# goktug97/estorch

Measured on NVIDIA H100. Metric: generations/sec at pop=4096, 1M-param MLP, higher is better.
Workload: dtype f32 (fp32-equivalent: evaluate GEMMs on wgmma with fp16 operands = 11-bit significand, TF32 class, each weight formed in fp32 from fp32 theta + the exactly-16-bit noise value and rounded once, f32 accumulate, f32 bias/loss; f32 ranks, reduction, Adam)

## Files before the change

estorch_b200/csrc/estk_eval_mlp_tc.cu:

```cuda
#include "estk_tc.cuh"
#include <type_traits>

namespace {

constexpr int kRows = 64;
constexpr int kTileN = 128;
constexpr int kHBlockBytes = kRows * kBlockK * 2;
constexpr int kHBytes = (kMaxW / kBlockK) * kHBlockBytes;
constexpr int kStageBytes = kTileN * kBlockK * 2;
constexpr int kStages = 5;
constexpr int kCluster = 4;
constexpr int kProdWarps = 8, kProdGroups = 4, kProdGroupWarps = kProdWarps / kProdGroups;
constexpr int kPT = 32 * kProdGroupWarps;
constexpr int kThreadsTC = 128 + 32 * kProdWarps;
static_assert(kProdGroups <= kStages, "parity waits need kProdGroups <= kStages");
constexpr int kItemsPT = kTileN / kCluster * (kBlockK / 8) / kPT;
constexpr int kTgtBatch = 4;
constexpr int kModeBF16 = 0, kModeBF16S = 1, kModeF16 = 2;

struct EvalTCParams {
  estk_mlp_desc desc;
  const float* theta;
  const float* table;
  const uint16_t* theta16;
  const uint16_t* table16;
  const int64_t* offsets;
  const int32_t* order;
  int pairs;
  float sigma;
  const float* obs;
  const float* target;
  int B, chunks;
  float* ret_plus;
  float* ret_minus;
  float* bc_plus;
  float* bc_minus;
  int bc_obs, bc_dim;
  float* partial;
  unsigned int* counters;
  float* centre_out;
  int n_centre;
  int n_tasks;
  int n_signs;
  int mode;
#ifdef ESTK_TC_PROFILE
  unsigned long long* prof;
#endif
};

#ifdef ESTK_TC_PROFILE
enum { kPrFull, kPrMma, kPrDrain, kPrLayer, kPrTask, kPrLoad, kPrEmpty, kPrForm, kPrBuckets };
unsigned long long* g_prof_buf = nullptr;
#define ESTK_PROF_DECL long long pr_[kPrBuckets] = {}; long long pr_t_ = clock64();
#define ESTK_PROF(b) do { const long long n_ = clock64(); pr_[b] += n_ - pr_t_; pr_t_ = n_; } while (0)
#else
#define ESTK_PROF_DECL
#define ESTK_PROF(b) do {} while (0)
#endif

struct Layer { int K, N; int64_t wbase, bbase; };

struct TaskId { int slot, sgn, chunk; bool centre; };
__device__ __forceinline__ TaskId decode_task(const EvalTCParams& p, int task, bool all_centre) {
  TaskId t;
  if (task < p.n_centre) { t.slot = 0; t.sgn = 0; t.chunk = task; t.centre = true; return t; }
  const int q = task - p.n_centre;
  t.chunk = q % p.chunks;
  t.sgn = (q / p.chunks) % p.n_signs;
  t.slot = q / (p.chunks * p.n_signs);
  t.centre = all_centre;
  return t;
}

template <int MODE>
__global__ void __launch_bounds__(kThreadsTC, 1) eval_mlp_tc_kernel(const EvalTCParams p) {
  constexpr bool S16 = (MODE == kModeBF16S), F16 = (MODE == kModeF16);
  extern __shared__ __align__(1024) uint8_t smem_raw[];
  uint8_t* smem = reinterpret_cast<uint8_t*>((reinterpret_cast<uintptr_t>(smem_raw) + 1023) & ~uintptr_t(1023));
  uint8_t* sH = smem;
  uint8_t* sB = sH + 2 * kHBytes;
  float* sBias = reinterpret_cast<float*>(sB + kStages * kStageBytes);
  uint64_t* bar_full = reinterpret_cast<uint64_t*>(sBias + kMaxW);
  uint64_t* bar_empty = bar_full + kStages;
  float* s_loss = reinterpret_cast<float*>(bar_empty + kStages);
  __shared__ Layer lay[ESTK_MAX_LAYERS];

  const int warp = threadIdx.x >> 5, lane = threadIdx.x & 31;
  const int L = p.desc.n_layers;
  if (threadIdx.x == 0) {
    for (int s = 0; s < kStages; ++s) {
      mbar_init(smem_u32(bar_full + s), 1);
      mbar_init(smem_u32(bar_empty + s), 4 * kCluster);
    }
    fence_barrier_init();
    int64_t pb = 0;
    for (int l = 0; l < L; ++l) {
      lay[l].K = p.desc.dims[l];
      lay[l].N = p.desc.dims[l + 1];
      lay[l].wbase = pb;
      lay[l].bbase = pb + (int64_t)lay[l].K * lay[l].N;
      pb = lay[l].bbase + lay[l].N;
    }
  }
  cluster_sync();
  const bool centre = (p.offsets == nullptr);
  ESTK_PROF_DECL

  if (warp < 4) {
    const int tid = threadIdx.x;
    const int r0 = warp * 16 + (lane >> 2);
    const int cq = (lane & 3) * 2;
    uint32_t kst = 0;
    for (int task = blockIdx.x; task < p.n_tasks; task += gridDim.x) {
      const TaskId tk = decode_task(p, task, centre);
      const int chunk = tk.chunk, sgn = tk.sgn, slot = tk.slot;
      const int j = (!tk.centre && p.order) ? p.order[slot] : slot;
      const float* trow = tk.centre ? p.theta : p.table + p.offsets[j];
      const float ssig = tk.centre ? 0.f : (sgn ? -p.sigma : p.sigma);
      float* bc = (tk.centre && !centre) ? nullptr : (sgn ? p.bc_minus : p.bc_plus);
      {
        const int K0 = lay[0].K, per_row = K0 / 8;
        for (int it = tid; it < kRows * per_row; it += 128) {
          const int r = it / per_row, c = it % per_row;
          const float* src = p.obs + (size_t)(chunk * kRows + r) * K0 + c * 8;
          const float4 x0 = __ldg(reinterpret_cast<const float4*>(src));
          const float4 x1 = __ldg(reinterpret_cast<const float4*>(src + 4));
          const uint32_t addr = smem_u32(sH + (c >> 3) * kHBlockBytes) + sw128_offset(r, c & 7);
          const uint32_t h0 = pack16<F16>(x0.x, x0.y), h1 = pack16<F16>(x0.z, x0.w);
          const uint32_t h2 = pack16<F16>(x1.x, x1.y), h3 = pack16<F16>(x1.z, x1.w);
          st_shared_v4(addr, h0, h1, h2, h3);
          if constexpr (F16) {
            const float2 f0 = unpack_f16(h0), f1 = unpack_f16(h1), f2 = unpack_f16(h2), f3 = unpack_f16(h3);
            st_shared_v4(addr + (K0 / kBlockK) * kHBlockBytes, pack_f16(x0.x - f0.x, x0.y - f0.y),
                         pack_f16(x0.z - f1.x, x0.w - f1.y), pack_f16(x1.x - f2.x, x1.y - f2.y),
                         pack_f16(x1.z - f3.x, x1.w - f3.y));
          }
        }
      }
      ESTK_PROF(kPrTask);
      float loss = 0.f;
      for (int l = 0; l < L; ++l) {
        const int K = lay[l].K, N = lay[l].N;
        const bool last = (l == L - 1);
        const uint32_t h_in = smem_u32(sH + (l & 1) * kHBytes);
        const uint32_t h_out = smem_u32(sH + ((l + 1) & 1) * kHBytes);
        named_bar_sync(1, 128);
        {
          float bz[kMaxW / 128], bt[kMaxW / 128];
#pragma unroll
          for (int i = 0; i < kMaxW / 128; ++i) {
            const int o = tid + i * 128;
            if (o < N) {
              bz[i] = ld_noise1(trow + lay[l].bbase + o);
              bt[i] = __ldg(p.theta + lay[l].bbase + o);
            }
          }
#pragma unroll
          for (int i = 0; i < kMaxW / 128; ++i)
            if (tid + i * 128 < N) sBias[tid + i * 128] = fmaf(ssig, bz[i], bt[i]);
        }
        fence_proxy_async();
        named_bar_sync(1, 128);
        ESTK_PROF(kPrLayer);
        const int lo_kb = (F16 && l == 0) ? K / kBlockK : 0;
        for (int n0 = 0; n0 < N; n0 += kTileN) {
          const int width = min(kTileN, N - n0);
          float d[64];
          uint32_t prev = 0;
          auto k_loop = [&](auto np_tag) {
            constexpr int NP = decltype(np_tag)::value;
            for (int kb = 0; kb < K / kBlockK; ++kb, ++kst) {
              const uint32_t stage = kst % kStages, phase = (kst / kStages) & 1u;
              mbar_wait(smem_u32(bar_full + stage), phase);
              ESTK_PROF(kPrFull);
              const uint32_t a_addr = h_in + kb * kHBlockBytes, b_addr = smem_u32(sB + stage * kStageBytes);
              wgmma_fence();
#pragma unroll
              for (int pass = 0; pass < NP; ++pass) {
                const uint32_t a = a_addr + pass * lo_kb * kHBlockBytes;
#pragma unroll
                for (int k = 0; k < kBlockK / 16; ++k)
                  wgmma_m64n128k16<F16>(d, make_sw128_desc(a + k * 32), make_sw128_desc(b_addr + k * 32),
                                        (kb | k | pass) != 0 ? 1u : 0u);
              }
              wgmma_commit();
              wgmma_wait<1>();
              if (kb > 0 && lane < kCluster) mbar_arrive_cluster(mapa_shared(smem_u32(bar_empty + prev), lane));
              prev = stage;
              ESTK_PROF(kPrMma);
            }
          };
          if (F16 && lo_kb) k_loop(std::integral_constant<int, 2>{});
          else k_loop(std::integral_constant<int, 1>{});
          wgmma_wait<0>();
          fence_acc(d);
          if (lane < kCluster) mbar_arrive_cluster(mapa_shared(smem_u32(bar_empty + prev), lane));
          if (last) {
#pragma unroll
            for (int jg = 0; jg < kTileN / 8; jg += kTgtBatch) {
              float2 t[kTgtBatch][2];
#pragma unroll
              for (int jb = jg; jb < jg + kTgtBatch; ++jb)
#pragma unroll
                for (int h = 0; h < 2; ++h)
                  if (jb * 8 < width)
                    t[jb - jg][h] = __ldg(reinterpret_cast<const float2*>(
                        p.target + (size_t)(chunk * kRows + r0 + 8 * h) * N + n0 + jb * 8 + cq));
#pragma unroll
              for (int jb = jg; jb < jg + kTgtBatch; ++jb) {
                if (jb * 8 < width) {
                  const int col = n0 + jb * 8 + cq;
                  const float2 bv = *reinterpret_cast<const float2*>(sBias + col);
#pragma unroll
                  for (int h = 0; h < 2; ++h) {
                    const int b = chunk * kRows + r0 + 8 * h;
                    const float y0 = d[jb * 4 + 2 * h] + bv.x, y1 = d[jb * 4 + 2 * h + 1] + bv.y;
                    const float e0 = y0 - t[jb - jg][h].x, e1 = y1 - t[jb - jg][h].y;
                    loss = fmaf(e0, e0, loss);
                    loss = fmaf(e1, e1, loss);
                    if (bc && b < p.bc_obs) {
                      const int64_t idx = (int64_t)b * N + col;
                      if (idx < p.bc_dim) bc[(size_t)j * p.bc_dim + idx] = y0;
                      if (idx + 1 < p.bc_dim) bc[(size_t)j * p.bc_dim + idx + 1] = y1;
                    }
                  }
                }
              }
            }
          } else {
#pragma unroll
            for (int jb = 0; jb < kTileN / 8; ++jb) {
              if (jb * 8 < width) {
                const int col = n0 + jb * 8 + cq;
                const float2 bv = *reinterpret_cast<const float2*>(sBias + col);
#pragma unroll
                for (int h = 0; h < 2; ++h) {
                  const int r = r0 + 8 * h;
                  const float y0 = d[jb * 4 + 2 * h] + bv.x, y1 = d[jb * 4 + 2 * h + 1] + bv.y;
                  st_shared_u32(h_out + (col >> 6) * kHBlockBytes + sw128_offset(r, (col & 63) >> 3) + (col & 7) * 2,
                                pack16_relu<F16>(y0, y1));
                }
              }
            }
          }
          ESTK_PROF(kPrDrain);
        }
      }
      loss = warp_sum_f(loss);
      if (lane == 0) s_loss[warp] = loss;
      named_bar_sync(1, 128);
      if (tid == 0) {
        const float tot = (s_loss[0] + s_loss[1]) + (s_loss[2] + s_loss[3]);
        const int parts = p.chunks;
        const bool folded = tk.centre && !centre;
        const int cell = folded ? p.pairs * 2 : slot * 2 + sgn;
        float* part = p.partial + (size_t)cell * parts;
        part[chunk] = tot;
        __threadfence();
        const unsigned int arrived = atomicAdd(p.counters + cell, 1u);
        if (arrived == (unsigned int)parts - 1) {
          __threadfence();
          float s = 0.f;
          for (int c = 0; c < parts; ++c) s += __ldcg(part + c);
          const float r = -(s / ((float)p.B * (float)lay[L - 1].N));
          if (folded) p.centre_out[0] = r;
          else if (sgn) p.ret_minus[j] = r;
          else p.ret_plus[j] = r;
          p.counters[cell] = 0u;
        }
      }
      ESTK_PROF(kPrTask);
    }
  } else {
    const int pwarp = warp - 4;
    const int pgroup = pwarp / kProdGroupWarps;
    const int ptid = (pwarp % kProdGroupWarps) * 32 + lane;
    const uint32_t rank = cluster_ctarank();
    int cached_task = -1;
    const float* trow = p.theta;
    const uint16_t* trow16 = nullptr;
    float ssig = 0.f;
    int task = blockIdx.x, l = 0, n0 = 0, kb = 0;
    auto advance = [&]() -> bool {
      if (++kb >= lay[l].K / kBlockK) {
        kb = 0;
        n0 += kTileN;
        if (n0 >= lay[l].N) {
          n0 = 0;
          if (++l == L) { l = 0; task += gridDim.x; }
        }
      }
      return task < p.n_tasks;
    };
    bool has = task < p.n_tasks;
    for (int sk = 0; sk < pgroup && has; ++sk) has = advance();
    uint32_t kst = pgroup;
    while (has) {
      if (task != cached_task) {
        cached_task = task;
        const TaskId tk = decode_task(p, task, centre);
        const int jj = (!tk.centre && p.order) ? p.order[tk.slot] : tk.slot;
        trow = tk.centre ? p.theta : p.table + p.offsets[jj];
        trow16 = tk.centre ? (S16 ? p.theta16 : nullptr) : p.table16 + p.offsets[jj];
        ssig = tk.centre ? 0.f : (tk.sgn ? -p.sigma : p.sigma);
      }
      const uint32_t stage = kst % kStages, phase = (kst / kStages) & 1u;
      const uint32_t sbase = smem_u32(sB + stage * kStageBytes);
      const int K = lay[l].K;
      const int qrows = min(kTileN, lay[l].N - n0) / kCluster;
      const int n_items = qrows * 8;
      const uint32_t qbase = sbase + rank * qrows * 128, qbytes = qrows * 128;
      const int64_t rbase = lay[l].wbase + (int64_t)(n0 + rank * qrows) * K + kb * kBlockK;
      {
        float4 th[kItemsPT][2], ep[kItemsPT][2];
        uint4 t16[kItemsPT], e16[kItemsPT];
#pragma unroll
        for (int u = 0; u < kItemsPT; ++u) {
          const int it = u * kPT + ptid;
          if (it < n_items) {
            const int64_t off = rbase + (int64_t)(it >> 3) * K + (it & 7) * 8;
            if constexpr (S16) {
              t16[u] = ld_noise4u(reinterpret_cast<const uint4*>(p.theta16 + off));
              e16[u] = ld_noise4u(reinterpret_cast<const uint4*>(trow16 + off));
            } else if constexpr (F16) {
              th[u][0] = ld_noise4(reinterpret_cast<const float4*>(p.theta + off));
              th[u][1] = ld_noise4(reinterpret_cast<const float4*>(p.theta + off + 4));
              e16[u] = trow16 ? ld_noise4u(reinterpret_cast<const uint4*>(trow16 + off)) : make_uint4(0u, 0u, 0u, 0u);
            } else {
              th[u][0] = ld_noise4(reinterpret_cast<const float4*>(p.theta + off));
              th[u][1] = ld_noise4(reinterpret_cast<const float4*>(p.theta + off + 4));
              ep[u][0] = ld_noise4(reinterpret_cast<const float4*>(trow + off));
              ep[u][1] = ld_noise4(reinterpret_cast<const float4*>(trow + off + 4));
            }
          }
        }
#ifdef ESTK_TC_PROFILE
        uint32_t ready = 0;
#pragma unroll
        for (int u = 0; u < kItemsPT; ++u) {
          if constexpr (S16) ready ^= t16[u].x ^ e16[u].x;
          else if constexpr (F16) ready ^= __float_as_uint(th[u][1].w) ^ e16[u].x;
          else ready ^= __float_as_uint(th[u][1].w) ^ __float_as_uint(ep[u][1].w);
        }
        if (ready == 0x7fc00001u) pr_[kPrForm] -= 1;
        ESTK_PROF(kPrLoad);
#endif
        mbar_wait(smem_u32(bar_empty + stage), phase ^ 1);
        ESTK_PROF(kPrEmpty);
#pragma unroll
        for (int u = 0; u < kItemsPT; ++u) {
          const int it = u * kPT + ptid;
          if (it < n_items) {
            const float sg = ssig;
            uint32_t w[4];
            if constexpr (S16) {
              const uint32_t sg2 = pack_bf16(sg, sg);
              const uint32_t tw[4] = {t16[u].x, t16[u].y, t16[u].z, t16[u].w};
              const uint32_t ew[4] = {e16[u].x, e16[u].y, e16[u].z, e16[u].w};
#pragma unroll
              for (int c = 0; c < 4; ++c) asm("fma.rn.bf16x2 %0, %1, %2, %3;" : "=r"(w[c]) : "r"(sg2), "r"(ew[c]), "r"(tw[c]));
            } else if constexpr (F16) {
              const float2 e0 = unpack_f16(e16[u].x), e1 = unpack_f16(e16[u].y);
              const float2 e2 = unpack_f16(e16[u].z), e3 = unpack_f16(e16[u].w);
              w[0] = pack_f16(fmaf(sg, e0.x, th[u][0].x), fmaf(sg, e0.y, th[u][0].y));
              w[1] = pack_f16(fmaf(sg, e1.x, th[u][0].z), fmaf(sg, e1.y, th[u][0].w));
              w[2] = pack_f16(fmaf(sg, e2.x, th[u][1].x), fmaf(sg, e2.y, th[u][1].y));
              w[3] = pack_f16(fmaf(sg, e3.x, th[u][1].z), fmaf(sg, e3.y, th[u][1].w));
            } else {
              w[0] = pack_bf16(fmaf(sg, ep[u][0].x, th[u][0].x), fmaf(sg, ep[u][0].y, th[u][0].y));
              w[1] = pack_bf16(fmaf(sg, ep[u][0].z, th[u][0].z), fmaf(sg, ep[u][0].w, th[u][0].w));
              w[2] = pack_bf16(fmaf(sg, ep[u][1].x, th[u][1].x), fmaf(sg, ep[u][1].y, th[u][1].y));
              w[3] = pack_bf16(fmaf(sg, ep[u][1].z, th[u][1].z), fmaf(sg, ep[u][1].w, th[u][1].w));
            }
            st_shared_v4(qbase + sw128_offset(it >> 3, it & 7), w[0], w[1], w[2], w[3]);
          }
        }
      }
      fence_proxy_async();
      named_bar_sync(2 + pgroup, kPT);
      if (ptid == 0) {
        const uint32_t full = smem_u32(bar_full + stage);
        mbar_arrive_expect_tx(full, (kCluster - 1) * qbytes);
        for (uint32_t r = 1; r < kCluster; ++r) {
          const uint32_t peer = (rank + r) % kCluster;
          bulk_copy_to_cluster(mapa_shared(qbase, peer), qbase, qbytes, mapa_shared(full, peer));
        }
      }
      for (int sk = 0; sk < kProdGroups && has; ++sk) has = advance();
      kst += kProdGroups;
      ESTK_PROF(kPrForm);
    }
  }
#ifdef ESTK_TC_PROFILE
  if (lane == 0 && p.prof) {
    unsigned long long* o = p.prof + ((size_t)blockIdx.x * (blockDim.x / 32) + warp) * kPrBuckets;
    for (int b = 0; b < kPrBuckets; ++b) o[b] = (unsigned long long)pr_[b];
  }
#endif
  cluster_sync();
}

size_t tc_smem_bytes() {
  return 1024 + 2 * (size_t)kHBytes + (size_t)kStages * kStageBytes + kMaxW * sizeof(float) +
         2 * kStages * sizeof(uint64_t) + 4 * sizeof(float);
}

template <int MODE>
int launch_tc(const EvalTCParams& p, cudaStream_t stream) {
  const size_t smem = tc_smem_bytes();
  ESTK_CUDA(cudaFuncSetAttribute(eval_mlp_tc_kernel<MODE>, cudaFuncAttributeMaxDynamicSharedMemorySize, (int)smem));
  cudaLaunchAttribute attr[1];
  attr[0].id = cudaLaunchAttributeClusterDimension;
  attr[0].val.clusterDim.x = kCluster;
  attr[0].val.clusterDim.y = 1;
  attr[0].val.clusterDim.z = 1;
  cudaLaunchConfig_t cfg = {};
  cfg.gridDim = dim3(kCluster);
  cfg.blockDim = dim3(kThreadsTC);
  cfg.dynamicSmemBytes = smem;
  cfg.stream = stream;
  cfg.attrs = attr;
  cfg.numAttrs = 1;
  int clusters = 0;
  ESTK_CUDA(cudaOccupancyMaxActiveClusters(&clusters, eval_mlp_tc_kernel<MODE>, &cfg));
  if (clusters < 1) {
    estk_set_error("eval_mlp_tc_kernel: no cluster of %d CTAs fits on this device", kCluster);
    return ESTK_ERR_CUDA;
  }
  const int items = p.n_tasks / kCluster;
  cfg.gridDim = dim3(kCluster * (clusters < items ? clusters : items));
  ESTK_CUDA(cudaLaunchKernelEx(&cfg, eval_mlp_tc_kernel<MODE>, p));
  return ESTK_OK;
}

int tc_supported(const estk_mlp_desc& d, int B, const char** why, int mode) {
  if (mode == kModeF16 && d.n_layers >= 1 && 2 * d.dims[0] > kMaxW) {
    *why = "fp16 mode splits the observations into hi + lo halves: input width <= 256"; return 0;
  }
  if (d.n_layers < 1 || d.n_layers > ESTK_MAX_LAYERS) { *why = "n_layers"; return 0; }
  if (d.activation != 0) { *why = "activation"; return 0; }
  for (int l = 0; l < d.n_layers; ++l) {
    if (d.dims[l] % 64 || d.dims[l] > kMaxW || d.dims[l] < 64) { *why = "layer input width must be a multiple of 64 in [64,512]"; return 0; }
    const int N = d.dims[l + 1];
    if (N % 32 || N > kMaxW || N < 32) { *why = "layer output width must be a multiple of 32 in [32,512]"; return 0; }
  }
  if (B % 256) { *why = "batch must be a multiple of 256"; return 0; }
  return 1;
}

int run_tc(estk_ctx* ctx, EvalTCParams& p, cudaStream_t stream, const char* who) {
  const char* why = "";
  if (!tc_supported(p.desc, p.B, &why, p.mode)) {
    estk_set_error("%s: shape not supported by the tensor-core path (%s)", who, why);
    return ESTK_ERR_UNSUPPORTED;
  }
  ESTK_CHECK_ARG(p.pairs >= 1 && p.pairs <= ESTK_MAX_POPULATION / 2, "%s: pairs=%d", who, p.pairs);
  p.chunks = p.B / kRows;
  ESTK_CHECK_ARG(p.chunks <= 2 * kEvalMaxChunks, "%s: batch too large", who);
  p.n_centre = p.centre_out ? p.chunks : 0;
  ESTK_CHECK_ARG(!p.centre_out || p.pairs * 2 < ESTK_MAX_POPULATION, "%s: population too large to fold the centre task", who);
  p.n_tasks = p.n_centre + p.pairs * p.n_signs * p.chunks;
  p.partial = ctx->eval_partial;
  p.counters = ctx->counters;
#ifdef ESTK_TC_PROFILE
  p.prof = g_prof_buf;
#endif
  if (p.mode == kModeF16) return launch_tc<kModeF16>(p, stream);
  if (p.mode == kModeBF16S) return launch_tc<kModeBF16S>(p, stream);
  return launch_tc<kModeBF16>(p, stream);
}

}

extern "C" int estk_eval_mlp_bf16(estk_ctx* ctx, const estk_mlp_desc* desc, const float* theta,
                                  const float* table, const int64_t* offsets, const int32_t* order,
                                  int32_t pairs, float sigma, const float* obs, const float* target,
                                  int32_t B, float* returns_plus, float* returns_minus, float* bc_plus,
                                  float* bc_minus, int32_t bc_obs, int32_t bc_dim, float* centre_return_out,
                                  void* stream) {
  ESTK_CHECK_ARG(ctx && desc && theta && table && offsets && obs && target && returns_plus && returns_minus,
                 "estk_eval_mlp_bf16: null argument");
  ESTK_CHECK_ARG((bc_plus == nullptr) == (bc_minus == nullptr), "estk_eval_mlp_bf16: bc_plus/bc_minus must both be set or both null");
  ESTK_CHECK_ARG(ESTK_ALIGNED16(theta) && ESTK_ALIGNED16(table) && ESTK_ALIGNED16(obs) && ESTK_ALIGNED16(target),
                 "estk_eval_mlp_bf16: theta/table/obs/target must be 16-byte aligned");
  EvalTCParams p = {};
  p.desc = *desc; p.theta = theta; p.table = table; p.offsets = offsets; p.order = order;
  p.pairs = pairs; p.sigma = sigma; p.obs = obs; p.target = target; p.B = B;
  p.ret_plus = returns_plus; p.ret_minus = returns_minus;
  p.bc_plus = bc_plus; p.bc_minus = bc_minus; p.bc_obs = bc_obs; p.bc_dim = bc_dim;
  p.n_signs = 2; p.centre_out = centre_return_out; p.mode = kModeBF16;
  return run_tc(ctx, p, (cudaStream_t)stream, "estk_eval_mlp_bf16");
}

extern "C" int estk_eval_mlp_center_bf16(estk_ctx* ctx, const estk_mlp_desc* desc, const float* theta,
                                         const float* obs, const float* target, int32_t B,
                                         float* return_out, float* bc_out, int32_t bc_obs,
                                         int32_t bc_dim, void* stream) {
  ESTK_CHECK_ARG(ctx && desc && theta && obs && target && return_out, "estk_eval_mlp_center_bf16: null argument");
  EvalTCParams p = {};
  p.desc = *desc; p.theta = theta; p.table = theta; p.offsets = nullptr; p.order = nullptr;
  p.pairs = 1; p.sigma = 0.f; p.obs = obs; p.target = target; p.B = B;
  p.ret_plus = return_out; p.ret_minus = nullptr;
  p.bc_plus = bc_out; p.bc_minus = nullptr; p.bc_obs = bc_obs; p.bc_dim = bc_dim;
  p.n_signs = 1; p.mode = kModeBF16;
  return run_tc(ctx, p, (cudaStream_t)stream, "estk_eval_mlp_center_bf16");
}

__global__ void __launch_bounds__(256) shadow_bf16_kernel(const float4* __restrict__ src, uint2* __restrict__ dst, int64_t n4) {
  const int64_t stride = (int64_t)gridDim.x * blockDim.x;
  for (int64_t i = (int64_t)blockIdx.x * blockDim.x + threadIdx.x; i < n4; i += stride) {
    const float4 v = src[i];
    uint2 o;
    asm("cvt.rn.bf16x2.f32 %0, %1, %2;" : "=r"(o.x) : "f"(v.y), "f"(v.x));
    asm("cvt.rn.bf16x2.f32 %0, %1, %2;" : "=r"(o.y) : "f"(v.w), "f"(v.z));
    dst[i] = o;
  }
}

extern "C" int estk_shadow_bf16(estk_ctx* ctx, const float* src, uint16_t* dst, int64_t n, void* stream) {
  ESTK_CHECK_ARG(ctx && src && dst && n > 0 && (n % 4) == 0, "estk_shadow_bf16: null argument or n not a multiple of 4");
  ESTK_CHECK_ARG(ESTK_ALIGNED16(src) && ((uintptr_t)dst & 7u) == 0, "estk_shadow_bf16: unaligned buffers");
  int blocks = (int)((n / 4 + 255) / 256);
  if (blocks > ctx->sm_count * 16) blocks = ctx->sm_count * 16;
  shadow_bf16_kernel<<<blocks, 256, 0, (cudaStream_t)stream>>>(reinterpret_cast<const float4*>(src),
                                                             reinterpret_cast<uint2*>(dst), n / 4);
  ESTK_CUDA(cudaGetLastError());
  return ESTK_OK;
}

extern "C" int estk_eval_mlp_bf16s(estk_ctx* ctx, const estk_mlp_desc* desc, const float* theta,
                                   const uint16_t* theta16, const float* table, const uint16_t* table16,
                                   const int64_t* offsets, const int32_t* order, int32_t pairs, float sigma,
                                   const float* obs, const float* target, int32_t B, float* returns_plus,
                                   float* returns_minus, float* bc_plus, float* bc_minus, int32_t bc_obs,
                                   int32_t bc_dim, float* centre_return_out, void* stream) {
  ESTK_CHECK_ARG(ctx && desc && theta && theta16 && table && table16 && offsets && obs && target &&
                 returns_plus && returns_minus, "estk_eval_mlp_bf16s: null argument");
  ESTK_CHECK_ARG((bc_plus == nullptr) == (bc_minus == nullptr), "estk_eval_mlp_bf16s: bc_plus/bc_minus must both be set or both null");
  ESTK_CHECK_ARG(ESTK_ALIGNED16(theta) && ESTK_ALIGNED16(table) && ESTK_ALIGNED16(obs) && ESTK_ALIGNED16(target) &&
                 ESTK_ALIGNED16(theta16) && ESTK_ALIGNED16(table16),
                 "estk_eval_mlp_bf16s: buffers must be 16-byte aligned");
  EvalTCParams p = {};
  p.desc = *desc; p.theta = theta; p.table = table; p.theta16 = theta16; p.table16 = table16;
  p.offsets = offsets; p.order = order;
  p.pairs = pairs; p.sigma = sigma; p.obs = obs; p.target = target; p.B = B;
  p.ret_plus = returns_plus; p.ret_minus = returns_minus;
  p.bc_plus = bc_plus; p.bc_minus = bc_minus; p.bc_obs = bc_obs; p.bc_dim = bc_dim;
  p.n_signs = 2; p.centre_out = centre_return_out; p.mode = kModeBF16S;
  return run_tc(ctx, p, (cudaStream_t)stream, "estk_eval_mlp_bf16s");
}

extern "C" int estk_eval_mlp_center_bf16s(estk_ctx* ctx, const estk_mlp_desc* desc, const float* theta,
                                          const uint16_t* theta16, const float* obs, const float* target,
                                          int32_t B, float* return_out, float* bc_out, int32_t bc_obs,
                                          int32_t bc_dim, void* stream) {
  ESTK_CHECK_ARG(ctx && desc && theta && theta16 && obs && target && return_out, "estk_eval_mlp_center_bf16s: null argument");
  EvalTCParams p = {};
  p.desc = *desc; p.theta = theta; p.table = theta; p.theta16 = theta16; p.table16 = theta16;
  p.offsets = nullptr; p.order = nullptr;
  p.pairs = 1; p.sigma = 0.f; p.obs = obs; p.target = target; p.B = B;
  p.ret_plus = return_out; p.ret_minus = nullptr;
  p.bc_plus = bc_out; p.bc_minus = nullptr; p.bc_obs = bc_obs; p.bc_dim = bc_dim;
  p.n_signs = 1; p.mode = kModeBF16S;
  return run_tc(ctx, p, (cudaStream_t)stream, "estk_eval_mlp_center_bf16s");
}

__global__ void __launch_bounds__(256) shadow_f16_kernel(const float4* __restrict__ src, uint2* __restrict__ dst, int64_t n4,
                                                         unsigned long long* __restrict__ inexact) {
  const int64_t stride = (int64_t)gridDim.x * blockDim.x;
  unsigned int bad = 0;
  for (int64_t i = (int64_t)blockIdx.x * blockDim.x + threadIdx.x; i < n4; i += stride) {
    const float4 v = src[i];
    const __half2 a = __floats2half2_rn(v.x, v.y), b = __floats2half2_rn(v.z, v.w);
    const float2 fa = __half22float2(a), fb = __half22float2(b);
    bad += (fa.x != v.x) + (fa.y != v.y) + (fb.x != v.z) + (fb.y != v.w);
    uint2 o;
    o.x = *reinterpret_cast<const uint32_t*>(&a);
    o.y = *reinterpret_cast<const uint32_t*>(&b);
    dst[i] = o;
  }
  if (inexact && bad) atomicAdd(inexact, (unsigned long long)bad);
}

extern "C" int estk_shadow_f16(estk_ctx* ctx, const float* src, uint16_t* dst, int64_t n, uint64_t* inexact_count,
                               void* stream) {
  ESTK_CHECK_ARG(ctx && src && dst && n > 0 && (n % 4) == 0, "estk_shadow_f16: null argument or n not a multiple of 4");
  ESTK_CHECK_ARG(ESTK_ALIGNED16(src) && ((uintptr_t)dst & 7u) == 0, "estk_shadow_f16: unaligned buffers");
  int blocks = (int)((n / 4 + 255) / 256);
  if (blocks > ctx->sm_count * 16) blocks = ctx->sm_count * 16;
  shadow_f16_kernel<<<blocks, 256, 0, (cudaStream_t)stream>>>(reinterpret_cast<const float4*>(src),
                                                            reinterpret_cast<uint2*>(dst), n / 4,
                                                            reinterpret_cast<unsigned long long*>(inexact_count));
  ESTK_CUDA(cudaGetLastError());
  return ESTK_OK;
}

extern "C" int estk_eval_mlp_f16(estk_ctx* ctx, const estk_mlp_desc* desc, const float* theta, const float* table,
                                 const uint16_t* table16, const int64_t* offsets, const int32_t* order, int32_t pairs,
                                 float sigma, const float* obs, const float* target, int32_t B, float* returns_plus,
                                 float* returns_minus, float* bc_plus, float* bc_minus, int32_t bc_obs,
                                 int32_t bc_dim, float* centre_return_out, void* stream) {
  ESTK_CHECK_ARG(ctx && desc && theta && table && table16 && offsets && obs && target && returns_plus && returns_minus,
                 "estk_eval_mlp_f16: null argument");
  ESTK_CHECK_ARG((bc_plus == nullptr) == (bc_minus == nullptr), "estk_eval_mlp_f16: bc_plus/bc_minus must both be set or both null");
  ESTK_CHECK_ARG(ESTK_ALIGNED16(theta) && ESTK_ALIGNED16(table) && ESTK_ALIGNED16(obs) && ESTK_ALIGNED16(target) &&
                 ESTK_ALIGNED16(table16), "estk_eval_mlp_f16: buffers must be 16-byte aligned");
  EvalTCParams p = {};
  p.desc = *desc; p.theta = theta; p.table = table; p.table16 = table16;
  p.offsets = offsets; p.order = order;
  p.pairs = pairs; p.sigma = sigma; p.obs = obs; p.target = target; p.B = B;
  p.ret_plus = returns_plus; p.ret_minus = returns_minus;
  p.bc_plus = bc_plus; p.bc_minus = bc_minus; p.bc_obs = bc_obs; p.bc_dim = bc_dim;
  p.n_signs = 2; p.centre_out = centre_return_out; p.mode = kModeF16;
  return run_tc(ctx, p, (cudaStream_t)stream, "estk_eval_mlp_f16");
}

extern "C" int estk_eval_mlp_center_f16(estk_ctx* ctx, const estk_mlp_desc* desc, const float* theta,
                                        const float* obs, const float* target, int32_t B, float* return_out,
                                        float* bc_out, int32_t bc_obs, int32_t bc_dim, void* stream) {
  ESTK_CHECK_ARG(ctx && desc && theta && obs && target && return_out, "estk_eval_mlp_center_f16: null argument");
  ESTK_CHECK_ARG(ESTK_ALIGNED16(theta) && ESTK_ALIGNED16(obs) && ESTK_ALIGNED16(target),
                 "estk_eval_mlp_center_f16: buffers must be 16-byte aligned");
  EvalTCParams p = {};
  p.desc = *desc; p.theta = theta; p.table = theta; p.offsets = nullptr; p.order = nullptr;
  p.pairs = 1; p.sigma = 0.f; p.obs = obs; p.target = target; p.B = B;
  p.ret_plus = return_out; p.ret_minus = nullptr;
  p.bc_plus = bc_out; p.bc_minus = nullptr; p.bc_obs = bc_obs; p.bc_dim = bc_dim;
  p.n_signs = 1; p.mode = kModeF16;
  return run_tc(ctx, p, (cudaStream_t)stream, "estk_eval_mlp_center_f16");
}

#ifdef ESTK_TC_PROFILE
extern "C" ESTK_API int estk_tc_profile(void* buf, int32_t* warps, int32_t* consumer_warps) {
  g_prof_buf = static_cast<unsigned long long*>(buf);
  *warps = kThreadsTC / 32;
  *consumer_warps = 4;
  return kPrBuckets;
}
#endif

extern "C" int estk_eval_mlp_f16_supported(const estk_mlp_desc* desc, int32_t B) {
  const char* why = "";
  return desc ? tc_supported(*desc, B, &why, kModeF16) : 0;
}

extern "C" int estk_eval_mlp_bf16_supported(const estk_mlp_desc* desc, int32_t B) {
  const char* why = "";
  return desc ? tc_supported(*desc, B, &why, kModeBF16) : 0;
}
```

estorch_b200/csrc/estk_tc.cuh:

```cuda
#pragma once
#include "estk_common.cuh"
#include <cuda_bf16.h>
#include <cuda_fp16.h>

namespace {

constexpr int kMaxW = 512;
constexpr int kBlockK = 64;

__device__ __forceinline__ uint32_t smem_u32(const void* p) {
  return (uint32_t)__cvta_generic_to_shared(p);
}
__device__ __forceinline__ void mbar_init(uint32_t bar, uint32_t count) {
  asm volatile("mbarrier.init.shared::cta.b64 [%0], %1;" ::"r"(bar), "r"(count));
}
__device__ __forceinline__ void mbar_wait(uint32_t bar, uint32_t parity) {
  asm volatile(
      "{\n"
      ".reg .pred P1;\n"
      "LAB_WAIT:\n"
      "mbarrier.try_wait.parity.shared::cta.b64 P1, [%0], %1;\n"
      "@P1 bra DONE;\n"
      "bra LAB_WAIT;\n"
      "DONE:\n"
      "}" ::"r"(bar), "r"(parity) : "memory");
}
__device__ __forceinline__ void fence_barrier_init() { asm volatile("fence.mbarrier_init.release.cluster;" ::: "memory"); }

__device__ __forceinline__ uint32_t cluster_ctarank() {
  uint32_t r;
  asm volatile("mov.u32 %0, %%cluster_ctarank;" : "=r"(r));
  return r;
}
__device__ __forceinline__ void cluster_sync() {
  asm volatile("barrier.cluster.arrive.release.aligned;\nbarrier.cluster.wait.acquire.aligned;" ::: "memory");
}
__device__ __forceinline__ uint32_t mapa_shared(uint32_t addr, uint32_t rank) {
  uint32_t r;
  asm volatile("mapa.shared::cluster.u32 %0, %1, %2;" : "=r"(r) : "r"(addr), "r"(rank));
  return r;
}
__device__ __forceinline__ void mbar_arrive_cluster(uint32_t bar) {
  asm volatile("mbarrier.arrive.shared::cluster.b64 _, [%0];" ::"r"(bar) : "memory");
}
__device__ __forceinline__ void mbar_arrive_expect_tx(uint32_t bar, uint32_t bytes) {
  asm volatile("mbarrier.arrive.expect_tx.shared::cta.b64 _, [%0], %1;" ::"r"(bar), "r"(bytes) : "memory");
}
__device__ __forceinline__ void bulk_copy_to_cluster(uint32_t dst, uint32_t src, uint32_t bytes, uint32_t bar) {
  asm volatile("cp.async.bulk.shared::cluster.shared::cta.mbarrier::complete_tx::bytes [%0], [%1], %2, [%3];"
               ::"r"(dst), "r"(src), "r"(bytes), "r"(bar) : "memory");
}
__device__ __forceinline__ void fence_proxy_async() { asm volatile("fence.proxy.async.shared::cta;" ::: "memory"); }

__device__ __forceinline__ uint4 ld_noise4u(const uint4* p) {
  uint4 v;
  asm volatile("ld.global.nc.L1::no_allocate.v4.u32 {%0,%1,%2,%3}, [%4];" : "=r"(v.x), "=r"(v.y), "=r"(v.z), "=r"(v.w) : "l"(p));
  return v;
}

__device__ __forceinline__ uint64_t make_sw128_desc(uint32_t smem_addr) {
  return (uint64_t)((smem_addr >> 4) & 0x3FFFu) | (1ull << 16) | ((uint64_t)(1024 >> 4) << 32) | (1ull << 62);
}
__device__ __forceinline__ uint32_t sw128_offset(int r, int c8) {
  return (uint32_t)((r >> 3) * 1024 + (r & 7) * 128 + ((c8 ^ (r & 7)) << 4));
}
__device__ __forceinline__ void wgmma_fence() { asm volatile("wgmma.fence.sync.aligned;" ::: "memory"); }
__device__ __forceinline__ void wgmma_commit() { asm volatile("wgmma.commit_group.sync.aligned;" ::: "memory"); }
template <int N> __device__ __forceinline__ void wgmma_wait() {
  asm volatile("wgmma.wait_group.sync.aligned %0;" ::"n"(N) : "memory");
}
__device__ __forceinline__ void fence_acc(float (&d)[64]) {
#pragma unroll
  for (int i = 0; i < 64; ++i) asm volatile("" : "+f"(d[i])::"memory");
}
template <bool F16>
__device__ __forceinline__ void wgmma_m64n128k16(float (&d)[64], uint64_t da, uint64_t db, uint32_t accumulate) {
#define ESTK_WG_D8(i) "+f"(d[i]), "+f"(d[i + 1]), "+f"(d[i + 2]), "+f"(d[i + 3]), "+f"(d[i + 4]), "+f"(d[i + 5]), "+f"(d[i + 6]), "+f"(d[i + 7])
#define ESTK_WG_ASM(TYPE)                                                                                        \
  asm volatile(                                                                                                  \
      "{\n.reg .pred p;\nsetp.ne.b32 p, %66, 0;\n"                                                                \
      "wgmma.mma_async.sync.aligned.m64n128k16.f32." TYPE "." TYPE " "                                           \
      "{%0,%1,%2,%3,%4,%5,%6,%7,%8,%9,%10,%11,%12,%13,%14,%15,%16,%17,%18,%19,%20,%21,%22,%23,%24,%25,%26,%27,"  \
      "%28,%29,%30,%31,%32,%33,%34,%35,%36,%37,%38,%39,%40,%41,%42,%43,%44,%45,%46,%47,%48,%49,%50,%51,%52,%53," \
      "%54,%55,%56,%57,%58,%59,%60,%61,%62,%63}, %64, %65, p, 1, 1, 0, 0;\n}"                                     \
      : ESTK_WG_D8(0), ESTK_WG_D8(8), ESTK_WG_D8(16), ESTK_WG_D8(24), ESTK_WG_D8(32), ESTK_WG_D8(40),            \
        ESTK_WG_D8(48), ESTK_WG_D8(56)                                                                           \
      : "l"(da), "l"(db), "r"(accumulate))
  if constexpr (F16) ESTK_WG_ASM("f16");
  else ESTK_WG_ASM("bf16");
#undef ESTK_WG_ASM
#undef ESTK_WG_D8
}
__device__ __forceinline__ uint32_t pack_bf16(float lo, float hi) {
  uint32_t r;
  asm("cvt.rn.bf16x2.f32 %0, %1, %2;" : "=r"(r) : "f"(hi), "f"(lo));
  return r;
}
__device__ __forceinline__ uint32_t pack_bf16_relu(float lo, float hi) {
  uint32_t r;
  asm("cvt.rn.relu.bf16x2.f32 %0, %1, %2;" : "=r"(r) : "f"(hi), "f"(lo));
  return r;
}
__device__ __forceinline__ uint32_t pack_f16(float lo, float hi) {
  uint32_t r;
  asm("cvt.rn.satfinite.f16x2.f32 %0, %1, %2;" : "=r"(r) : "f"(hi), "f"(lo));
  return r;
}
__device__ __forceinline__ uint32_t pack_f16_relu(float lo, float hi) {
  uint32_t r;
  asm("cvt.rn.relu.satfinite.f16x2.f32 %0, %1, %2;" : "=r"(r) : "f"(hi), "f"(lo));
  return r;
}
__device__ __forceinline__ float2 unpack_f16(uint32_t h2) {
  return __half22float2(*reinterpret_cast<const __half2*>(&h2));
}
template <bool F16> __device__ __forceinline__ uint32_t pack16(float lo, float hi) {
  return F16 ? pack_f16(lo, hi) : pack_bf16(lo, hi);
}
template <bool F16> __device__ __forceinline__ uint32_t pack16_relu(float lo, float hi) {
  return F16 ? pack_f16_relu(lo, hi) : pack_bf16_relu(lo, hi);
}
__device__ __forceinline__ void st_shared_v4(uint32_t addr, uint32_t a, uint32_t b, uint32_t c, uint32_t d) {
  asm volatile("st.shared.v4.b32 [%0], {%1,%2,%3,%4};" ::"r"(addr), "r"(a), "r"(b), "r"(c), "r"(d) : "memory");
}
__device__ __forceinline__ uint4 ld_shared_v4u(uint32_t addr) {
  uint4 v;
  asm volatile("ld.shared.v4.u32 {%0,%1,%2,%3}, [%4];" : "=r"(v.x), "=r"(v.y), "=r"(v.z), "=r"(v.w) : "r"(addr));
  return v;
}
__device__ __forceinline__ float4 ld_shared_v4(uint32_t addr) {
  float4 v;
  asm volatile("ld.shared.v4.f32 {%0,%1,%2,%3}, [%4];" : "=f"(v.x), "=f"(v.y), "=f"(v.z), "=f"(v.w) : "r"(addr));
  return v;
}
__device__ __forceinline__ void named_bar_sync(int id, int threads) {
  asm volatile("bar.sync %0, %1;" ::"r"(id), "r"(threads) : "memory");
}
__device__ __forceinline__ void st_shared_u32(uint32_t addr, uint32_t v) {
  asm volatile("st.shared.b32 [%0], %1;" ::"r"(addr), "r"(v) : "memory");
}


}
```

Before: 87.12.

## Add second consumer warpgroup ping-ponging N tiles with setmaxnreg register split

Adds a second 128-thread consumer warpgroup that takes alternating N tiles, so one group's epilogue (bias, loss, target loads) overlaps the other's wgmma mainloop. The groups order their mainloops with named barriers, pass the running loss through shared memory, and use a double-buffered bias array. setmaxnreg moves registers from the producer warps to the consumers, and the target batch size is halved to lower register pressure. The added cross-group barriers and the tighter producer register budget could cause stalls or spills.

```diff
diff --git a/estorch_b200/csrc/estk_eval_mlp_tc.cu b/estorch_b200/csrc/estk_eval_mlp_tc.cu
--- a/estorch_b200/csrc/estk_eval_mlp_tc.cu
+++ b/estorch_b200/csrc/estk_eval_mlp_tc.cu
@@ -12,10 +12,14 @@
 constexpr int kCluster = 4;
 constexpr int kProdWarps = 8, kProdGroups = 4, kProdGroupWarps = kProdWarps / kProdGroups;
 constexpr int kPT = 32 * kProdGroupWarps;
-constexpr int kThreadsTC = 128 + 32 * kProdWarps;
+constexpr int kConsWG = 2, kConsThreads = 128 * kConsWG;
+constexpr int kThreadsTC = kConsThreads + 32 * kProdWarps;
+constexpr int kConsRegs = 152, kProdRegs = 104;
+static_assert(kConsRegs + kProdRegs <= 256, "setmaxnreg split exceeds the register file");
+constexpr int kBarCons = 1, kBarOrder = 6, kBarLoss = 8, kBarWG = 10;
 static_assert(kProdGroups <= kStages, "parity waits need kProdGroups <= kStages");
 constexpr int kItemsPT = kTileN / kCluster * (kBlockK / 8) / kPT;
-constexpr int kTgtBatch = 4;
+constexpr int kTgtBatch = 2;
 constexpr int kModeBF16 = 0, kModeBF16S = 1, kModeF16 = 2;
 
 struct EvalTCParams {
@@ -49,7 +53,7 @@
 };
 
 #ifdef ESTK_TC_PROFILE
-enum { kPrFull, kPrMma, kPrDrain, kPrLayer, kPrTask, kPrLoad, kPrEmpty, kPrForm, kPrBuckets };
+enum { kPrFull, kPrMma, kPrDrain, kPrLayer, kPrTask, kPrOther, kPrLoad, kPrEmpty, kPrForm, kPrBuckets };
 unsigned long long* g_prof_buf = nullptr;
 #define ESTK_PROF_DECL long long pr_[kPrBuckets] = {}; long long pr_t_ = clock64();
 #define ESTK_PROF(b) do { const long long n_ = clock64(); pr_[b] += n_ - pr_t_; pr_t_ = n_; } while (0)
@@ -80,9 +84,10 @@
   uint8_t* sH = smem;
   uint8_t* sB = sH + 2 * kHBytes;
   float* sBias = reinterpret_cast<float*>(sB + kStages * kStageBytes);
-  uint64_t* bar_full = reinterpret_cast<uint64_t*>(sBias + kMaxW);
+  uint64_t* bar_full = reinterpret_cast<uint64_t*>(sBias + 2 * kMaxW);
   uint64_t* bar_empty = bar_full + kStages;
   float* s_loss = reinterpret_cast<float*>(bar_empty + kStages);
+  float* s_chain = s_loss + 4;
   __shared__ Layer lay[ESTK_MAX_LAYERS];
 
   const int warp = threadIdx.x >> 5, lane = threadIdx.x & 31;
@@ -106,21 +111,28 @@
   const bool centre = (p.offsets == nullptr);
   ESTK_PROF_DECL
 
-  if (warp < 4) {
-    const int tid = threadIdx.x;
-    const int r0 = warp * 16 + (lane >> 2);
+  if (warp < 4 * kConsWG) {
+    setmaxnreg_inc<kConsRegs>();
+    const int cw = warp >> 2;
+    const int ctid = threadIdx.x;
+    const int tid = ctid & 127;
+    const int r0 = (warp & 3) * 16 + (lane >> 2);
     const int cq = (lane & 3) * 2;
     uint32_t kst = 0;
+    bool mine = (cw == 0);
+    bool after = (cw != 0);
     for (int task = blockIdx.x; task < p.n_tasks; task += gridDim.x) {
       const TaskId tk = decode_task(p, task, centre);
       const int chunk = tk.chunk, sgn = tk.sgn, slot = tk.slot;
       const int j = (!tk.centre && p.order) ? p.order[slot] : slot;
       const float* trow = tk.centre ? p.theta : p.table + p.offsets[j];
       const float ssig = tk.centre ? 0.f : (sgn ? -p.sigma : p.sigma);
-      float* bc = (tk.centre && !centre) ? nullptr : (sgn ? p.bc_minus : p.bc_plus);
+      const bool with_bc = !(tk.centre && !centre) && p.bc_plus;
+      const bool final_task = task + (int)gridDim.x >= p.n_tasks;
+      named_bar_sync(kBarCons, kConsThreads);
       {
         const int K0 = lay[0].K, per_row = K0 / 8;
-        for (int it = tid; it < kRows * per_row; it += 128) {
+        for (int it = ctid; it < kRows * per_row; it += kConsThreads) {
           const int r = it / per_row, c = it % per_row;
           const float* src = p.obs + (size_t)(chunk * kRows + r) * K0 + c * 8;
           const float4 x0 = __ldg(reinterpret_cast<const float4*>(src));
@@ -144,27 +156,35 @@
         const bool last = (l == L - 1);
         const uint32_t h_in = smem_u32(sH + (l & 1) * kHBytes);
         const uint32_t h_out = smem_u32(sH + ((l + 1) & 1) * kHBytes);
-        named_bar_sync(1, 128);
+        float* bias = sBias + (l & 1) * kMaxW;
         {
-          float bz[kMaxW / 128], bt[kMaxW / 128];
-#pragma unroll
-          for (int i = 0; i < kMaxW / 128; ++i) {
-            const int o = tid + i * 128;
+          float bz[kMaxW / kConsThreads], bt[kMaxW / kConsThreads];
+#pragma unroll
+          for (int i = 0; i < kMaxW / kConsThreads; ++i) {
+            const int o = ctid + i * kConsThreads;
             if (o < N) {
               bz[i] = ld_noise1(trow + lay[l].bbase + o);
               bt[i] = __ldg(p.theta + lay[l].bbase + o);
             }
           }
 #pragma unroll
-          for (int i = 0; i < kMaxW / 128; ++i)
-            if (tid + i * 128 < N) sBias[tid + i * 128] = fmaf(ssig, bz[i], bt[i]);
+          for (int i = 0; i < kMaxW / kConsThreads; ++i)
+            if (ctid + i * kConsThreads < N) bias[ctid + i * kConsThreads] = fmaf(ssig, bz[i], bt[i]);
         }
         fence_proxy_async();
-        named_bar_sync(1, 128);
+        named_bar_sync(kBarCons, kConsThreads);
         ESTK_PROF(kPrLayer);
         const int lo_kb = (F16 && l == 0) ? K / kBlockK : 0;
-        for (int n0 = 0; n0 < N; n0 += kTileN) {
+        for (int n0 = 0; n0 < N; n0 += kTileN, mine = !mine) {
+          if (!mine) {
+            kst += K / kBlockK;
+            continue;
+          }
           const int width = min(kTileN, N - n0);
+          const bool last_tile = n0 + kTileN >= N;
+          if (after) named_bar_sync(kBarOrder + cw, kConsThreads);
+          after = true;
+          ESTK_PROF(kPrOther);
           float d[64];
           uint32_t prev = 0;
           auto k_loop = [&](auto np_tag) {
@@ -192,6 +212,7 @@
           };
           if (F16 && lo_kb) k_loop(std::integral_constant<int, 2>{});
           else k_loop(std::integral_constant<int, 1>{});
+          if (!(last && last_tile && final_task)) named_bar_arrive(kBarOrder + (cw ^ 1), kConsThreads);
           wgmma_wait<0>();
           fence_acc(d);
           if (lane < kCluster) mbar_arrive_cluster(mapa_shared(smem_u32(bar_empty + prev), lane));
@@ -206,11 +227,17 @@
                   if (jb * 8 < width)
                     t[jb - jg][h] = __ldg(reinterpret_cast<const float2*>(
                         p.target + (size_t)(chunk * kRows + r0 + 8 * h) * N + n0 + jb * 8 + cq));
+              if (jg == 0 && n0 > 0) {
+                ESTK_PROF(kPrDrain);
+                named_bar_sync(kBarLoss + cw, kConsThreads);
+                loss = s_chain[tid];
+                ESTK_PROF(kPrOther);
+              }
 #pragma unroll
               for (int jb = jg; jb < jg + kTgtBatch; ++jb) {
                 if (jb * 8 < width) {
                   const int col = n0 + jb * 8 + cq;
-                  const float2 bv = *reinterpret_cast<const float2*>(sBias + col);
+                  const float2 bv = *reinterpret_cast<const float2*>(bias + col);
 #pragma unroll
                   for (int h = 0; h < 2; ++h) {
                     const int b = chunk * kRows + r0 + 8 * h;
@@ -218,7 +245,8 @@
                     const float e0 = y0 - t[jb - jg][h].x, e1 = y1 - t[jb - jg][h].y;
                     loss = fmaf(e0, e0, loss);
                     loss = fmaf(e1, e1, loss);
-                    if (bc && b < p.bc_obs) {
+                    if (with_bc && b < p.bc_obs) {
+                      float* bc = sgn ? p.bc_minus : p.bc_plus;
                       const int64_t idx = (int64_t)b * N + col;
                       if (idx < p.bc_dim) bc[(size_t)j * p.bc_dim + idx] = y0;
                       if (idx + 1 < p.bc_dim) bc[(size_t)j * p.bc_dim + idx + 1] = y1;
@@ -227,12 +255,16 @@
                 }
               }
             }
+            if (!last_tile) {
+              s_chain[tid] = loss;
+              named_bar_arrive(kBarLoss + (cw ^ 1), kConsThreads);
+            }
           } else {
 #pragma unroll
             for (int jb = 0; jb < kTileN / 8; ++jb) {
               if (jb * 8 < width) {
                 const int col = n0 + jb * 8 + cq;
-                const float2 bv = *reinterpret_cast<const float2*>(sBias + col);
+                const float2 bv = *reinterpret_cast<const float2*>(bias + col);
 #pragma unroll
                 for (int h = 0; h < 2; ++h) {
                   const int r = r0 + 8 * h;
@@ -246,9 +278,10 @@
           ESTK_PROF(kPrDrain);
         }
       }
+      if (mine) continue;
       loss = warp_sum_f(loss);
-      if (lane == 0) s_loss[warp] = loss;
-      named_bar_sync(1, 128);
+      if (lane == 0) s_loss[warp & 3] = loss;
+      named_bar_sync(kBarWG + cw, 128);
       if (tid == 0) {
         const float tot = (s_loss[0] + s_loss[1]) + (s_loss[2] + s_loss[3]);
         const int parts = p.chunks;
@@ -272,11 +305,11 @@
       ESTK_PROF(kPrTask);
     }
   } else {
-    const int pwarp = warp - 4;
+    setmaxnreg_dec<kProdRegs>();
+    const int pwarp = warp - 4 * kConsWG;
     const int pgroup = pwarp / kProdGroupWarps;
     const int ptid = (pwarp % kProdGroupWarps) * 32 + lane;
-    const uint32_t rank = cluster_ctarank();
-    int cached_task = -1;
+    bool new_task = true;
     const float* trow = p.theta;
     const uint16_t* trow16 = nullptr;
     float ssig = 0.f;
@@ -287,7 +320,7 @@
         n0 += kTileN;
         if (n0 >= lay[l].N) {
           n0 = 0;
-          if (++l == L) { l = 0; task += gridDim.x; }
+          if (++l == L) { l = 0; task += gridDim.x; new_task = true; }
         }
       }
       return task < p.n_tasks;
@@ -296,8 +329,8 @@
     for (int sk = 0; sk < pgroup && has; ++sk) has = advance();
     uint32_t kst = pgroup;
     while (has) {
-      if (task != cached_task) {
-        cached_task = task;
+      if (new_task) {
+        new_task = false;
         const TaskId tk = decode_task(p, task, centre);
         const int jj = (!tk.centre && p.order) ? p.order[tk.slot] : tk.slot;
         trow = tk.centre ? p.theta : p.table + p.offsets[jj];
@@ -309,6 +342,7 @@
       const int K = lay[l].K;
       const int qrows = min(kTileN, lay[l].N - n0) / kCluster;
       const int n_items = qrows * 8;
+      const uint32_t rank = cluster_ctarank();
       const uint32_t qbase = sbase + rank * qrows * 128, qbytes = qrows * 128;
       const int64_t rbase = lay[l].wbase + (int64_t)(n0 + rank * qrows) * K + kb * kBlockK;
       {
@@ -377,7 +411,7 @@
         }
       }
       fence_proxy_async();
-      named_bar_sync(2 + pgroup, kPT);
+      named_bar_sync(2 + (int)(threadIdx.x / kPT) - kConsThreads / kPT, kPT);
       if (ptid == 0) {
         const uint32_t full = smem_u32(bar_full + stage);
         mbar_arrive_expect_tx(full, (kCluster - 1) * qbytes);
@@ -401,8 +435,8 @@
 }
 
 size_t tc_smem_bytes() {
-  return 1024 + 2 * (size_t)kHBytes + (size_t)kStages * kStageBytes + kMaxW * sizeof(float) +
-         2 * kStages * sizeof(uint64_t) + 4 * sizeof(float);
+  return 1024 + 2 * (size_t)kHBytes + (size_t)kStages * kStageBytes + 2 * kMaxW * sizeof(float) +
+         2 * kStages * sizeof(uint64_t) + (4 + 128) * sizeof(float);
 }
 
 template <int MODE>
@@ -634,7 +668,7 @@
 extern "C" ESTK_API int estk_tc_profile(void* buf, int32_t* warps, int32_t* consumer_warps) {
   g_prof_buf = static_cast<unsigned long long*>(buf);
   *warps = kThreadsTC / 32;
-  *consumer_warps = 4;
+  *consumer_warps = 4 * kConsWG;
   return kPrBuckets;
 }
 #endif
diff --git a/estorch_b200/csrc/estk_tc.cuh b/estorch_b200/csrc/estk_tc.cuh
--- a/estorch_b200/csrc/estk_tc.cuh
+++ b/estorch_b200/csrc/estk_tc.cuh
@@ -136,6 +136,15 @@
 __device__ __forceinline__ void named_bar_sync(int id, int threads) {
   asm volatile("bar.sync %0, %1;" ::"r"(id), "r"(threads) : "memory");
 }
+__device__ __forceinline__ void named_bar_arrive(int id, int threads) {
+  asm volatile("bar.arrive %0, %1;" ::"r"(id), "r"(threads) : "memory");
+}
+template <int R> __device__ __forceinline__ void setmaxnreg_inc() {
+  asm volatile("setmaxnreg.inc.sync.aligned.u32 %0;" ::"n"(R));
+}
+template <int R> __device__ __forceinline__ void setmaxnreg_dec() {
+  asm volatile("setmaxnreg.dec.sync.aligned.u32 %0;" ::"n"(R));
+}
 __device__ __forceinline__ void st_shared_u32(uint32_t addr, uint32_t v) {
   asm volatile("st.shared.b32 [%0], %1;" ::"r"(addr), "r"(v) : "memory");
 }
```

Measured after the change: 91.70, median of 6. +5.3%, better.
